# fperezgamonal/flownet2-tf

Measured on AMD Instinct MI355X. Metric: forward pairs/sec at 512x384 (FlowNet2), higher is better.
Workload: dtype f16x2 (split fp16 hi+lo operands, 3 fp16 MFMAs per product, fp32 accumulate); 1 GPU; FlowNet2 forward, batch=4 synthetic 512x384 pairs per GPU, seeded synthetic weights; pairs_per_gpu=4, parallelism=dp1 (no collective)

## Files before the change

flownet2-tf_amd/csrc/conv.hip:

```cpp
#include "conv_common.h"
#include <cstdlib>

namespace fn2 {

template <typename T, typename OutT, int TC, int WC, int WP>
__global__ void __launch_bounds__(256) conv_igemm_kernel(const ConvArgs p) {
  constexpr int CH = 16 / (int)sizeof(T);
  constexpr int BC = WC * TC * 16;
  constexpr int BP = WP * 64;
  constexpr int NT = 256;
  static_assert(WC * WP == 4, "4 waves per block");
  constexpr int NPR = BP / 64;
  constexpr int NWR = (BC * 4 + NT - 1) / NT;
  constexpr int WSWZ_BIT = (TC == 4) ? 5 : (TC == 2) ? 4 : 3;
  __shared__ uint4 lds[2][(BC + BP) * 4];

  const int tid = threadIdx.x, lane = tid & 63, wave = tid >> 6;
  const int wc = wave / WP, wp = wave % WP;
  const int cid = tid & 3;

  int pad_y = p.pad, pad_x = p.pad, oy_off = 0, ox_off = 0, osc = 1;
  const T* wgt = reinterpret_cast<const T*>(p.wgt);
  const int phase = blockIdx.z / p.splitk, split = blockIdx.z - phase * p.splitk;
  if (p.deconv) {
// ... 796 lines not shown
    plan->layout = 0; plan->cout_tile = 16; plan->kstep_elems = 64 / esz;
    plan->wgt_dtype = in_dtype == FN2_F16X2 ? FN2_F32 : in_dtype;
    return FN2_OK;
  }
  if (conv_fast_ok(in_dtype, cin_pad, cout)) {
    plan->layout = 1; plan->cout_tile = cout > 64 ? 128 : cout > 32 ? 64 : 32; plan->kstep_elems = 128 / esz;
    plan->wgt_dtype = in_dtype;
    return FN2_OK;
  }
  if (in_dtype == FN2_F16X2)
    return fail(FN2_ERR_UNSUPPORTED, "split-fp16 inputs need cin_pad %% 32 == 0 (LDS-DMA kernel); got %d", cin_pad);
  plan->layout = 0; plan->cout_tile = cout > 64 ? 128 : cout > 32 ? 64 : cout > 16 ? 32 : 16;
  plan->kstep_elems = 64 / esz; plan->wgt_dtype = in_dtype;
  return FN2_OK;
}

}

namespace fn2 {

static bool is_flow_head(const fn2_conv_desc* d) {
  return d->kind == 0 && d->out.c == 2 && d->kh == 3 && d->kw == 3 && d->stride == 1 && d->pad == 1 &&
         d->out.dtype == FN2_F32 && d->act == FN2_ACT_NONE;
}

static bool wants_bp64(const ConvArgs& a, int tile, int phases, int layout) {
  if (layout != 1 || (a.dbg & 32)) return false;
  if (tile < 128) return true;
  const char* e = getenv("FN2_BP64_MIN");
  const int min_blocks = e ? atoi(e) : 96;
  return cdiv(a.M, 64) * (long)(a.cout_pad / 128) * phases >= min_blocks;
}

static int build_args(const fn2_conv_desc* d, ConvArgs* out, int* tile_out, int* phases_out) {
  FN2_REQUIRE(d, "conv2d: null descriptor");
  int rc = check_view(&d->in, "conv2d input");
  if (rc) return rc;
  rc = check_view(&d->out, "conv2d output");
  if (rc) return rc;
  FN2_REQUIRE(d->wgt, "conv2d: null weights");
  FN2_REQUIRE((d->kind >= 0 && d->kind <= 3) || d->kind == 5,
              "conv2d: kind must be 0 (conv), 1 (deconv k4 s2 crop 1), 2 (stem row-run conv), 3 (transpose of a stride-2 conv) "
              "or 5 (deconv k4 s2 crop 1, column phases merged)");
  FN2_REQUIRE(d->in.n == d->out.n, "conv2d: batch mismatch");
  FN2_REQUIRE(d->up_src == nullptr || ((d->kind == 1 || d->kind == 5) && d->up_w != nullptr && d->up_c0 >= 0 &&
                                       d->up_c0 + 2 <= d->out.cs && !d->accumulate),
              "conv2d: up_src rides on a kind-1 / kind-5 transposed conv (up_w set, [up_c0, up_c0 + 2) inside the out buffer)");
  FN2_REQUIRE(d->cin_pad % 8 == 0 && d->cin_pad >= d->in.c, "conv2d: cin_pad must be a multiple of 8 >= Cin");
  FN2_REQUIRE(d->in.cs % 8 == 0 && d->in.c0 % 8 == 0, "conv2d: input channel stride/offset must be multiples of 8");
  if (d->kind != 2)
    FN2_REQUIRE(d->in.c0 + d->cin_pad <= d->in.cs, "conv2d: padded input channels exceed the buffer stride");
  const int esz = dtype_size(d->in.dtype);
  const int CH = 16 / esz;
  FN2_REQUIRE(d->kpad > 0 && d->kpad % (4 * CH) == 0, "conv2d: kpad must be a multiple of one k-step");
  fn2_conv_plan plan;
  rc = fn2_conv2d_plan(d->in.dtype, d->cin_pad, d->out.c, &plan);
  if (rc) return rc;
  const bool wfrag = d->wgt_layout == 2;
  if (wfrag)
    FN2_REQUIRE(plan.layout == 1 && plan.cout_tile >= 64 && d->in.dtype == FN2_F16X2 && d->kind != 2,
                "conv2d: wgt_layout 2 (fragment order) is for split-fp16 layers with more than 32 output channels");
  else
    FN2_REQUIRE(d->wgt_layout == plan.layout, "conv2d: wgt_layout %d does not match fn2_conv2d_plan (%d)", d->wgt_layout,
                plan.layout);
  const int tile = plan.cout_tile;
  FN2_REQUIRE(d->cout_pad % tile == 0 && d->cout_pad >= d->out.c, "conv2d: cout_pad must be a multiple of the cout tile");
  FN2_REQUIRE(d->act == FN2_ACT_NONE || d->act == FN2_ACT_LEAKY, "conv2d: bad activation");
  FN2_REQUIRE(d->out.dtype == d->in.dtype || d->out.dtype == FN2_F32 ||
                  (d->in.dtype == FN2_F32 && d->out.dtype == FN2_F16X2),
              "conv2d: output dtype must be the input dtype, fp32, or split-fp16 from an fp32 stem");
  if (d->in.dtype == FN2_F16X2) FN2_REQUIRE(d->in.cs % 8 == 0 && d->in.c0 % 8 == 0, "conv2d: split-fp16 views are group (8) aligned");
  if (d->out.dtype == FN2_F16X2) FN2_REQUIRE(d->out.cs % 8 == 0 && d->out.c0 % 8 == 0, "conv2d: split-fp16 views are group (8) aligned");

  ConvArgs& a = *out;
  a = ConvArgs{};
  a.KH_KW_hint = 0;
  a.wfrag = wfrag ? 1 : 0;
  a.merged = d->kind == 5 ? 1 : 0;
  a.in = d->in.data; a.wgt = d->wgt; a.bias = d->bias; a.out = d->out.data;
  a.N = d->in.n; a.H = d->in.h; a.W = d->in.w; a.in_cs = d->in.cs; a.in_c0 = d->in.c0;
// ... 109 lines not shown
  }
  a.kg = 1;
  if (d->wgt_layout == 1 && tile == 128 && !(a.dbg & 32)) {
    const char* e_kg = getenv("FN2_KG");
    if (!e_kg || atoi(e_kg) != 0) {
      const char* e3 = getenv("FN2_KG3_MAX");
      const char* e2 = getenv("FN2_KG2_MAX");
      const long blocks = (long)cdiv(a.M, 64) * (a.cout_pad / 128) * phases;
      if (blocks <= (e3 ? atoi(e3) : 0)) { a.bp64 = 1; a.kg = 3; }
      else if (blocks <= (e2 ? atoi(e2) : 95)) { a.bp64 = 1; a.kg = 2; }
    }
  }
  if (d->wgt_layout == 1 && tile == 128 && !(a.dbg & 32) && d->in.dtype == FN2_F16X2) {
    const char* e_lo = getenv("FN2_DEEP_MIN");
    const char* e_hi = getenv("FN2_DEEP_MAX");
    const long blocks = (long)cdiv(a.M, 64) * (a.cout_pad / 128) * phases;
    const int lo = e_lo ? atoi(e_lo) : 0, hi = e_hi ? atoi(e_hi) : -1;
    if (blocks >= lo && blocks <= hi) { a.bp64 = 3; a.kg = 1; }
  }
  if (d->wgt_layout == 1 && tile == 128 && a.bp64 == 1 && a.kg == 1) {
    const char* e_ring = getenv("FN2_RING_MAX");
    const int ring_max = e_ring ? atoi(e_ring) : 512;
    const long blocks = (long)cdiv(a.M, 64) * (a.cout_pad / 128) * phases;
    if ((a.dbg & 256) || (blocks >= 384 && blocks <= ring_max)) a.bp64 = 2;
    const char* e_rs = getenv("FN2_RING_SPLIT");
    if (e_rs && blocks >= atoi(e_rs) && blocks < 384) a.bp64 = 2;
  }
  *tile_out = tile;
  *phases_out = phases;
  return FN2_OK;
}

static int preferred_split(const ConvArgs& a, int tile, int phases) {
  if (a.merged) return 1;
  const int bp = tile == 128 ? (a.bp64 ? 64 : 128) : (a.bp64 ? 128 : 256);
  const long blocks = (long)cdiv(a.M, bp) * (a.cout_pad / tile) * phases;
  const char* e_min = getenv("FN2_SPLIT_MINBLOCKS");
  if (blocks >= (e_min ? atoi(e_min) : 384)) return 1;
  if (a.bp64 == 3) {
    const char* e_sl = getenv("FN2_DEEP_SLOTS");
    int s = (int)((e_sl ? atoi(e_sl) : 256) / blocks);
    const int maxs = a.ksteps / 16;
    if (s > maxs) s = maxs;
    if (s > 16) s = 16;
    if (s < 2) return 1;
    const int kper = cdiv(a.ksteps, s);
    return cdiv(a.ksteps, kper);
  }
  if (a.kg > 1) {
    const char* e_nos = getenv("FN2_KG_NOSPLIT");
    if (blocks >= (e_nos ? atoi(e_nos) : 96)) return 1;
    const char* e_sl = getenv("FN2_KG_SLOTS");
    int s = (int)((e_sl ? atoi(e_sl) : 256) / blocks);
    const int maxs = a.ksteps / (12 * a.kg);
    if (s > maxs) s = maxs;
    if (s > 16) s = 16;
    if (s < 2) return 1;
    const int kper = cdiv(a.ksteps, s);
    return cdiv(a.ksteps, kper);
  }
  const char* e = getenv("FN2_SPLIT_SLOTS");
  const char* e_rsl = getenv("FN2_RING_SPLIT_SLOTS");
  const int slots = (tile == 128 && a.bp64 == 2) ? (e_rsl ? atoi(e_rsl) : 512) : e ? atoi(e) : 640;
  int s = (int)(slots / blocks);
  const int maxs = a.ksteps / 8;
  if (s > maxs) s = maxs;
  if (s > 16) s = 16;
// ... 20 lines not shown
}

int fn2_conv2d_splits(const fn2_conv_desc* d) {
  ConvArgs a;
  int tile, phases;
  if (build_args(d, &a, &tile, &phases) != FN2_OK || is_flow_head(d)) return 1;
  int sk = preferred_split(a, tile, phases);
  while (sk > 1 && (d->workspace == nullptr || split_bytes(a, sk) > d->workspace_bytes)) --sk;
  if ((long)a.N * a.out_H * a.out_W * a.ws_cs >= (1L << 31)) sk = 1;
  if (sk > 1) {
    const int kper = cdiv(a.ksteps, sk);
    sk = cdiv(a.ksteps, kper);
    if (d->wgt_layout >= 1) sk = cdiv(a.ksteps / 2, cdiv(kper, 2));
  }
  return sk < 1 ? 1 : sk;
}

int fn2_conv2d_kernel_name(const fn2_conv_desc* d, char* name, int cap) {
  FN2_REQUIRE(name && cap > 0, "conv2d_kernel_name: no buffer");
  name[0] = 0;
  if (!d || d->wgt_layout < 1 || is_flow_head(d)) return FN2_OK;
  conv_name_sink() = ConvNameSink{name, cap};
  const int rc = fn2_conv2d(d, nullptr);
  conv_name_sink() = ConvNameSink{nullptr, 0};
  return rc;
}

int fn2_conv2d(const fn2_conv_desc* d, void* stream) {
  ConvArgs a;
  int tile, phases;
  int rc = build_args(d, &a, &tile, &phases);
  if (rc) return rc;
  hipStream_t s = (hipStream_t)stream;
  if (is_flow_head(d)) {
    int blocks = grid_for((long)a.M * 64, 256);
    if (d->in.dtype == FN2_F16X2 && a.M <= 4096 && !(a.dbg & 32768)) {
      a.dbg |= 16384;
      blocks = a.M;
    } else {
      a.dbg &= ~16384;
    }
    if (d->in.dtype == FN2_F32)
      hipLaunchKernelGGL(flow_head_kernel<float>, dim3(blocks), dim3(256), 0, s, a);
    else if (d->in.dtype == FN2_BF16)
      hipLaunchKernelGGL(flow_head_kernel<bf16_t>, dim3(blocks), dim3(256), 0, s, a);
    else if (d->in.dtype == FN2_F16)
      hipLaunchKernelGGL(flow_head_kernel<f16_t>, dim3(blocks), dim3(256), 0, s, a);
    else
      hipLaunchKernelGGL(flow_head_kernel<x2_t>, dim3(blocks), dim3(256), 0, s, a);
    FN2_CHECK_LAUNCH("flow_head");
    return FN2_OK;
  }
  int sk = preferred_split(a, tile, phases);
  while (sk > 1 && (d->workspace == nullptr || split_bytes(a, sk) > d->workspace_bytes)) --sk;
  if ((long)a.N * a.out_H * a.out_W * a.ws_cs >= (1L << 31)) sk = 1;
  if (sk > 1) {
    a.kper = cdiv(a.ksteps, sk);
    sk = cdiv(a.ksteps, a.kper);
  }
  if (sk > 1) {
    a.splitk = sk;
    a.ws = reinterpret_cast<float*>(d->workspace);
  }
  if (d->up_src != nullptr && d->kind == 5 && 2 * d->out.c == 32) {
    a.up_src = d->up_src; a.up_w = d->up_w; a.up_bias = d->up_bias; a.up_c0 = d->up_c0;
  }
// ... 248 lines not shown
```

flownet2-tf_amd/csrc/conv2.hip:

```cpp
#include "conv_common.h"

#include <type_traits>
#include <algorithm>
#include <utility>

#ifndef FN2_X2_ORDER
#define FN2_X2_ORDER 0
#endif
#ifndef FN2_CONV_ABLATE
#define FN2_CONV_ABLATE 0
#endif
#ifndef FN2_SETPRIO
#define FN2_SETPRIO 1
#endif

namespace fn2 {

typedef __attribute__((address_space(3))) void* lptr_t;

constexpr unsigned kOobOffset = 0x80000000u;

typedef int v4i_t __attribute__((ext_vector_type(4)));
typedef unsigned u32x4_t __attribute__((ext_vector_type(4)));

// ... 932 lines not shown
        for (int i = 0; i < 4; ++i) {
          const int row = i * 8 + rr;
          *reinterpret_cast<uint4*>(ob + (size_t)row * osc * p.out_cs) = *reinterpret_cast<const uint4*>(etl + row * ERS + ch * 4);
        }
      } else if (vec16 && cout_base + 15 < p.Cout) {
        store16<OutT>(po, v);
      } else {
#pragma unroll
        for (int q = 0; q < 16; ++q)
          if (cout_base + q < p.Cout) store_elem<OutT>(po + q, v[q]);
      }
      if (p.merged && p.up_src != nullptr && cout_base == 0 && ox < p.OW) {
        const int uy = toy * osc + oy_off, ux = ox * osc + ox_off + bsel;
        const int H2 = p.out_H >> 1, W2 = p.out_W >> 1;
        const int a = uy & 1, b = ux & 1, y = uy >> 1, x = ux >> 1;
        float r0 = p.up_bias ? p.up_bias[0] : 0.f, r1 = p.up_bias ? p.up_bias[1] : 0.f;
#pragma unroll
        for (int ty = 0; ty < 2; ++ty) {
          const int iy = y - 1 + a + ty, ky = 3 - a - 2 * ty;
          if (iy < 0 || iy >= H2) continue;
#pragma unroll
          for (int tx = 0; tx < 2; ++tx) {
            const int ix = x - 1 + b + tx, kx = 3 - b - 2 * tx;
            if (ix < 0 || ix >= W2) continue;
            const float2 sv = *reinterpret_cast<const float2*>(p.up_src + (((long)tn * H2 + iy) * W2 + ix) * 2);
            const float* ww = p.up_w + (ky * 4 + kx) * 4;
            r0 += sv.x * ww[0] + sv.y * ww[1];
            r1 += sv.x * ww[2] + sv.y * ww[3];
          }
        }
        OutT* pu = out + (((size_t)tn * p.out_H + uy) * p.out_W + ux) * p.out_cs + p.up_c0;
        store_elem<OutT>(pu, r0);
        store_elem<OutT>(pu + 1, r1);
      }
    }
  }
#endif
}

template <typename OutT, int NST>
__global__ void __launch_bounds__(256) conv_stem_kernel(const ConvArgs p, const int ntiles) {
#if defined(__HIP_DEVICE_COMPILE__)
  using T = x2_t;
  constexpr int ESZ = 4;
  constexpr int BC = 64, BP = 128, TCN = 2;
  __shared__ uint4 ldsA[NST][BC * 8];
  __shared__ uint4 ldsB[2][NST][BP * 8];
  const int tid = threadIdx.x, lane = tid & 63;
  const int wave = __builtin_amdgcn_readfirstlane(tid >> 6);
  const unsigned wrow_bytes = (unsigned)p.ksteps * 128u;
  const v4i_t rsrc_w = make_rsrc(p.wgt, (int)(p.cout_pad * wrow_bytes));
  const v4i_t rsrc_x = make_rsrc(p.in, p.in_bytes);
  const int lrow = lane >> 3, lphys = lane & 7;
  const int spt = p.cin_chunks >> 3;
#pragma unroll
  for (int st = 0; st < NST; ++st) {
    const int sc = st / p.KH, ky = st - sc * p.KH;
#pragma unroll
    for (int j = 0; j < 2; ++j) {
      const int row = wave * 16 + j * 8 + lrow;
      const unsigned woff = (unsigned)row * wrow_bytes + (unsigned)((lphys ^ ((row >> 1) & 7)) * 16);
      dma16(rsrc_w, &ldsA[st][(wave * 16 + j * 8) * 8], woff, (ky * spt + sc) * 128);
    }
  }
  auto issue_B = [&](int tile, int buf) {
#pragma unroll
// ... 526 lines not shown
        else if (a.wfrag == 2)
          hipLaunchKernelGGL((conv_igemm2_kernel<T, OutT, 4, 1, 1, 2, 3, 1, false, true, false>), grid, dim3(256), 0, s, a);
        else if (slab)
          hipLaunchKernelGGL((conv_igemm2_kernel<T, OutT, 4, 1, 1, 2, 2, 1, false, true, true>), grid, dim3(256), 0, s, a);
        else
          hipLaunchKernelGGL((conv_igemm2_kernel<T, OutT, 4, 1, 1, 2, 2, 1, false, true, false>), grid, dim3(256), 0, s, a);
      }
    } else {
      return fail(FN2_ERR_UNSUPPORTED, "conv fast path: fragment-order weights are split fp16 only");
    }
  } else if (tile == 128 && a.bp64 && a.kg == 3) FN2_LAUNCH2(cdiv(a.M, 64), a.cout_pad / 128, 768, 2, 2, 2, 1, 2, 3);
  else if (tile == 128 && a.bp64 && a.kg == 2) FN2_LAUNCH2(cdiv(a.M, 64), a.cout_pad / 128, 512, 2, 2, 2, 1, 2, 2);
  else if (tile == 128 && a.bp64 == 3) FN2_LAUNCH2(cdiv(a.M, 64), a.cout_pad / 128, 256, 2, 2, 2, 1, 6, 1);
  else if (tile == 128 && a.bp64 == 2) FN2_LAUNCH2(cdiv(a.M, 64), a.cout_pad / 128, 256, 2, 2, 2, 1, 3, 1);
  else if (tile == 128 && a.bp64) FN2_LAUNCH2(cdiv(a.M, 64), a.cout_pad / 128, 256, 2, 2, 2, 1, 2, 1);
  else if (tile == 128) FN2_LAUNCH2(cdiv(a.M, 128), a.cout_pad / 128, 256, 2, 2, 2, 2, 2, 1);
  else if (tile == 64 && a.bp64) FN2_LAUNCH2(cdiv(a.M, 128), a.cout_pad / 64, 256, 1, 4, 2, 1, 2, 1);
  else if (tile == 64) FN2_LAUNCH2(cdiv(a.M, 256), a.cout_pad / 64, 256, 1, 4, 2, 2, 2, 1);
  else if (a.bp64) FN2_LAUNCH2(cdiv(a.M, 128), a.cout_pad / 32, 256, 1, 4, 1, 1, 2, 1);
  else FN2_LAUNCH2(cdiv(a.M, 256), a.cout_pad / 32, 256, 1, 4, 1, 2, 2, 1);
#undef FN2_LAUNCH2
  FN2_CHECK_LAUNCH("conv_igemm2");
  return FN2_OK;
}

int launch_head5_strip(const ConvArgs& a, int blocks, hipStream_t s) {
  if (a.ksteps == 3) hipLaunchKernelGGL((head5_strip_kernel<1>), dim3(blocks), dim3(512), 0, s, a);
  else if (a.ksteps == 6) hipLaunchKernelGGL((head5_strip_kernel<2>), dim3(blocks), dim3(512), 0, s, a);
  else return fail(FN2_ERR_UNSUPPORTED, "flow_head5 strip form: %d channel lines (3 or 6)", a.ksteps);
  FN2_CHECK_LAUNCH("flow_head5_strip");
  return FN2_OK;
}

int launch_head5(const ConvArgs& a, int blocks, hipStream_t s) {
  hipLaunchKernelGGL((conv_igemm2_kernel<x2_t, float, 1, 4, 2, 2, 2, 1, false, false, false, true>), dim3(blocks, 1, 1), dim3(256), 0,
                     s, a);
  FN2_CHECK_LAUNCH("flow_head5");
  return FN2_OK;
}

bool conv_fast_ok(int in_dtype, int cin_pad, int cout) {
  const int esz = dtype_size(in_dtype);
  return cout > 2 && (cin_pad * esz) % 128 == 0;
}

int launch_conv_fast(const ConvArgs& a, int in_dtype, int out_dtype, int tile, int phases, hipStream_t s) {
  if (tile != 128 && tile != 64 && tile != 32) return fail(FN2_ERR_UNSUPPORTED, "conv fast path: cout tile %d", tile);
  if (in_dtype == FN2_F32) return launch2<float, float>(a, tile, phases, s);
  if (in_dtype == FN2_BF16) {
    if (out_dtype == FN2_BF16) return launch2<bf16_t, bf16_t>(a, tile, phases, s);
    return launch2<bf16_t, float>(a, tile, phases, s);
  }
  if (in_dtype == FN2_F16) {
    if (out_dtype == FN2_F16) return launch2<f16_t, f16_t>(a, tile, phases, s);
    return launch2<f16_t, float>(a, tile, phases, s);
  }
  if (out_dtype == FN2_F16X2) {
    if (launch_rowrun<x2_t>(a, tile, phases, s)) { FN2_CHECK_LAUNCH("conv_rowrun"); return FN2_OK; }
    if (launch_stem<x2_t>(a, tile, phases, s)) { FN2_CHECK_LAUNCH("conv_stem"); return FN2_OK; }
    if (launch_halo<x2_t>(a, tile, phases, s)) { FN2_CHECK_LAUNCH("conv_halo"); return FN2_OK; }
    if (a.merged) return fail(FN2_ERR_UNSUPPORTED, "conv2d kind 5: needs the halo kernel (input width a multiple of 128, no split-K)");
    return launch2<x2_t, x2_t>(a, tile, phases, s);
  }
  if (launch_halo<float>(a, tile, phases, s)) { FN2_CHECK_LAUNCH("conv_halo"); return FN2_OK; }
  if (a.merged) return fail(FN2_ERR_UNSUPPORTED, "conv2d kind 5: needs the halo kernel (input width a multiple of 128, no split-K)");
  return launch2<x2_t, float>(a, tile, phases, s);
// ... 4 lines not shown
```

flownet2-tf_amd/csrc/conv_common.h:

```cpp
#pragma once
#include "fn2_common.h"

namespace fn2 {

struct ConvArgs {
  const void* in;
  const void* wgt;
  const float* bias;
  void* out;
  int N, H, W, in_cs, in_c0;
  int cin_chunks;
  int KH, KW, stride, pad;
  int OH, OW;
  int M;
  int out_H, out_W, out_cs, out_c0, Cout;
  int ksteps;
  int cout_pad;
  int act;
  int deconv;
  int ph_pad0, ph_pad1;
  int kh_ph[2], kw_ph[2];
  int merged;
  int wmajor;
  int bp64;
  int KH_KW_hint;
  int kg;
  int h5_tx, h5_ty, h5_ring;
  int h5_tiles, h5_groups;
  const float* h5_wc;
  const float* h5_bc;
  int h5_rows;
  int fh_M, fh_z0;
  const float* fh_w;
  int fh_w1, fh_groups;
  const float* fh_bias;
  float* fh_out;
  int fh_out_cs, fh_out_c0;
  float fh_scale;
  const float* up_src; const float* up_w; const float* up_bias; int up_c0;
  int wfrag;
  int accum;
  int vec_ok;
  int splitk;
  int kper;
  float* ws;
  int ws_cs;
  float out_scale;
  int in_bytes;
  const void* mask_y;
  int mask_c0, mask_c1;
  int dbg;
};

__device__ __forceinline__ void fh_pixel(const x2_t* __restrict__ in, int H, int W, int in_cs, int in_c0, int groups,
                                         const float* __restrict__ wf0, const float* __restrict__ wf1,
// ... 56 lines not shown
#pragma unroll
        for (int q = 0; q < 16; ++q) v[q] += o[q];
      }
      if (mask) {
        float y[16];
        load16<OutT>(reinterpret_cast<const OutT*>(p.mask_y) + (po - out_base), y);
#pragma unroll
        for (int q = 0; q < 16; ++q)
          if (cout_base + q >= p.mask_c0 && cout_base + q < p.mask_c1) v[q] *= y[q] > 0.f ? 1.f : (y[q] < 0.f ? 0.1f : 0.55f);
      }
    } else {
#pragma unroll
      for (int q = 0; q < 16; ++q)
        if (cout_base + q < p.Cout) {
          if (p.accum) v[q] += load_elem<OutT>(po + q);
          v[q] = act_grad<OutT>(p, out_base, po + q, cout_base + q, v[q]);
        }
    }
  }
}

template <typename OutT>
__device__ __forceinline__ void store4(OutT* p, float a, float b, float c, float d) {
  const float v[4] = {a, b, c, d};
  store_vec<OutT, 4>(p, v);
}

struct ConvNameSink { char* buf; int cap; };
ConvNameSink& conv_name_sink();

int launch_conv_fast(const ConvArgs& a, int in_dtype, int out_dtype, int tile, int phases, hipStream_t s);
int launch_head5(const ConvArgs& a, int blocks, hipStream_t s);
int launch_head5_strip(const ConvArgs& a, int blocks, hipStream_t s);
bool conv_fast_ok(int in_dtype, int cin_pad, int cout);

}
```

flownet2-tf_amd/src/engine.py:

```python
import ctypes as C
import math
import os

import numpy as np
import torch

from . import _hip, netdefs, weights as W

_DT = {"f32": torch.float32, "bf16": torch.bfloat16, "f16": torch.float16, "f16x2": torch.float32}
_CODE = {"f32": _hip.FN2_F32, "bf16": _hip.FN2_BF16, "f16": _hip.FN2_F16, "f16x2": _hip.FN2_F16X2}
_TILE_ARGS = {128: "2, 2, 2, 2", 64: "1, 4, 2, 2", 32: "1, 4, 1, 2"}


def conv2_kernel_args(tile, m, cout_pad, phases, x2=True):
    dbg = int(os.environ.get("FN2_CONV_DBG", "0"))
    blocks64 = -(-m // 64) * (cout_pad // 128) * phases if tile == 128 else 0
    big = "FN2_M16_MIN" in os.environ and blocks64 >= max(int(os.environ["FN2_M16_MIN"]), 513)
    m16 = "true" if (x2 and not dbg & 512 and (dbg & 1024 or big)) else "false"
    full = dbg & 32
    if tile < 128:
        base = {64: "1, 4, 2, 2, 2, 1", 32: "1, 4, 1, 2, 2, 1"}[tile] if full else {64: "1, 4, 2, 1, 2, 1", 32: "1, 4, 1, 1, 2, 1"}[tile]
        return f"{base}, {m16}"
    blocks = -(-m // 64) * (cout_pad // 128) * phases
    if not full and int(os.environ.get("FN2_KG", "1")):
# ... 168 lines not shown
                eng._branch = self_.prev
        return _L()

    def _head_lane(self):
        hd = self._branch + 2
        return hd if (self._lanes_on and self._branch in (0, 1) and (self._lane_mask >> hd) & 1) else self._branch

    def _op(self, name, fn, *args, kernel=None):
        self.kernel_of.append(kernel if kernel is not None else fn.__name__.replace("fn2_", ""))
        self.ops.append((name, fn, args))
        self.branch_of.append(self._branch)

    def _conv(self, scope, spec, src, dst, up=None, up_after=None, defer_head=False):
        name, kind, k, stride, pad, cin, cout, act = spec
        sbuf, sc0, sc = src
        dbuf, dc0, dc = dst
        assert sc == cin and dc == cout, (scope, name, sc, cin, dc, cout)
        head_px = dbuf.shape[0] * dbuf.shape[1] * dbuf.shape[2]
        if (self.heads_as_gemm and kind == "conv" and cout == 2 and k == 3 and stride == 1 and pad == 1 and not act
                and dbuf.dtype == torch.float32 and head_px >= int(os.environ.get("FN2_HEAD_GEMM_MIN", "8192"))
                and self._head_gemm(scope, spec, src, dst, up)):
            return up is not None and bool(int(os.environ.get("FN2_FUSE_UPFLOW", "1")))
        wname = f"{scope}/{name}/weights"
        in_code = self._code(sbuf)
        esz = 2 if in_code in (_hip.FN2_BF16, _hip.FN2_F16) else 4
        cin_pad = _round_up(cin, 8)
        cin_line = _round_up(cin, 128 // esz)
        if sc0 + cin_line <= sbuf.shape[3] and _hip.conv_plan(in_code, cin_line, cout).layout == 1:
            cin_pad = cin_line
        plan = _hip.conv_plan(in_code, cin_pad, cout)
        tile, layout = plan.cout_tile, plan.layout
        merged = (kind != "conv" and self.compose_heads and cout == 16 and in_code == _hip.FN2_F16X2 and layout == 1
                  and tile == 32 and sbuf.shape[2] % 128 == 0 and bool(int(os.environ.get("FN2_DECONV_MERGED", "1"))))
        if kind == "conv":
            packed, cin_pad, cout_pad, kpad = W.pack_conv(self._w(wname), tile, plan.kstep_elems, cin_pad, layout)
        elif merged:
            packed, cin_pad, cout_pad, kpad = W.pack_deconv_merged(self._w(wname), tile, plan.kstep_elems, cin_pad, layout)
        else:
            packed, cin_pad, cout_pad, kpad = W.pack_deconv(self._w(wname), tile, plan.kstep_elems, cin_pad, layout)
        bias = self._bias(scope, name, kind, cout)
        out_scale = 1.0
        if plan.wgt_dtype == _hip.FN2_F16X2:
            wmax = float(abs(packed).max())
            if wmax > 0:
                k2 = int(math.floor(math.log2(1024.0 / wmax)))
                packed = packed * (2.0 ** k2)
                out_scale = 2.0 ** (-k2)
        wdev = W.packed_to_device(packed, plan.wgt_dtype, self.device)
        d = _hip.Fn2ConvDesc()
        d.inp = self._v(sbuf, sc, sc0)
        d.out = self._v(dbuf, dc, dc0)
        d.wgt = wdev.data_ptr()
        d.bias = bias.data_ptr() if bias is not None else None
        d.kind = 0 if kind == "conv" else (5 if merged else 1)
        d.kh = d.kw = k
        d.stride, d.pad = stride, pad
        d.act = _hip.ACT_LEAKY if act else _hip.ACT_NONE
        d.cin_pad, d.cout_pad, d.kpad = cin_pad, cout_pad, kpad
        d.wgt_layout = layout
        d.out_scale = out_scale
        frag = False
        if (self.fragment_weights and layout == 1 and tile >= int(os.environ.get("FN2_WREG_TILE_MIN", "128"))
                and plan.wgt_dtype == _hip.FN2_F16X2 and self._wants_fragments(d)):
            wdev = W.to_fragment_order(wdev)
            d.wgt, d.wgt_layout, frag = wdev.data_ptr(), 2, True
        self.keep += [d, wdev, bias]
        self.conv_descs.append(d)
        self.desc_branch.append(self._branch)
        up_rec = None
        if self._pending_head is not None and kind != "conv":
            hd = self._pending_head
            assert up_after is not None and hd.inp.data == d.inp.data and hd.inp.c0 == d.inp.c0, (scope, name)
            d.head = C.addressof(hd)
            self._pending_head = None
        if up_after is not None:
            assert kind != "conv" and (not merged or cout == 16)
            up_name, up_src, (ubuf, uc0, uc) = up_after
            assert ubuf is dbuf and uc == 2
            uw = W.to_device(self._w(f"{scope}/{up_name}/weights"), torch.float32, self.device)
            ub = self._bias(scope, up_name, "deconv", 2)
            d.up_src, d.up_w, d.up_bias, d.up_c0 = up_src.data_ptr(), uw.data_ptr(), (ub.data_ptr() if ub is not None else None), uc0
            uv = self._v(ubuf, uc, uc0)
            self.keep += [uw, ub, uv]
            up_rec = dict(scope=scope, name=up_name, kind="upflow", src=up_src, dst=up_after[2], w=uw, b=ub, view=uv)
        self.layers.append(dict(scope=scope, name=name, kind=d.kind, k=k, stride=stride, pad=pad, cin=cin, cout=cout,
                                act=bool(act), src=src, dst=dst, desc=d, w=wdev, b=bias, cin_pad=cin_pad,
                                cout_pad=cout_pad, kpad=kpad, layout=layout, tile=tile, kstep=plan.kstep_elems, frag=frag))
        if up_rec is not None:
            self.layers.append(up_rec)
        tn = _TNAME[self.dtype_name] if in_code == self.act_code else "float"
        if kind == "conv" and cout == 2 and k == 3 and stride == 1 and pad == 1:
            kern = f"flow_head_kernel<{tn}>"
# ... 735 lines not shown
```

flownet2-tf_amd/src/weights.py:

```python
import os

import numpy as np
import torch

from . import netdefs


def init_weights(model, seed=1234, flow_gain=0.25, bias_std=0.02, head_biases=None):
    if head_biases is None:
        head_biases = model != "FlowNetS_interp"
    rng = np.random.default_rng(seed)
    w = {}
    for scope, layers in netdefs.model_scopes(model):
        for (name, kind, k, stride, pad, cin, cout, act) in layers:
            if kind == "conv":
                fan_in = k * k * cin
                std = np.sqrt((2.0 if act else 1.0) / fan_in)
                if name.startswith("predict_flow"):
                    std *= flow_gain
                w[f"{scope}/{name}/weights"] = (rng.standard_normal((k, k, cin, cout)) * std).astype(np.float32)
                b = (rng.standard_normal((cout,)) * bias_std).astype(np.float32)
                if netdefs.has_bias(model, name, kind, not head_biases):
                    w[f"{scope}/{name}/biases"] = b
            else:
# ... 92 lines not shown
    cout_pad = _round_up(cout, cout_tile)
    kpad = _round_up(4 * cin_pad, kstep_elems)
    out = np.zeros((4, cout_pad, kpad), dtype)
    for a in range(2):
        for b in range(2):
            p = np.zeros((cout_pad, 4, cin_pad), dtype)
            for ty in range(2):
                for tx in range(2):
                    p[:cout, ty * 2 + tx, :cin] = w_hwoi[3 - a - 2 * ty, 3 - b - 2 * tx]
            ph = np.zeros((cout_pad, kpad), dtype)
            ph[:, :4 * cin_pad] = p.reshape(cout_pad, -1)
            out[a * 2 + b] = _permute_rows64(ph) if layout == 1 else ph
    return out, cin_pad, cout_pad, kpad


def pack_deconv_merged(w_hwoi, cout_tile, kstep_elems, cin_pad, layout=1, dtype=np.float32):
    kh, kw, cout, cin = w_hwoi.shape
    assert kh == 4 and kw == 4 and cout in (16, 32) and cin_pad >= cin and cin_pad % 8 == 0 and cout_tile == 32
    cout_pad = 2 * cout
    kpad = _round_up(6 * cin_pad, kstep_elems)
    out = np.zeros((2, cout_pad, kpad), dtype)
    for a in range(2):
        p = np.zeros((cout_pad, 6, cin_pad), dtype)
        for b in range(2):
            for ty in range(2):
                for tx in range(2):
                    p[b * cout:(b + 1) * cout, ty * 3 + b + tx, :cin] = w_hwoi[3 - a - 2 * ty, 3 - b - 2 * tx]
        ph = np.zeros((cout_pad, kpad), dtype)
        ph[:, :6 * cin_pad] = p.reshape(cout_pad, -1)
        out[a] = _permute_rows64(ph) if layout == 1 else ph
    return out, cin_pad, cout_pad, kpad


def pack_conv_transpose_s2(w_hwio, p, cout_tile, kstep_elems, cin_pad, layout, dtype=np.float32):
    k, _, ci, co = w_hwio.shape
    T = (k + 1) // 2
    cout_pad = _round_up(ci, cout_tile)
    kpad = _round_up(T * T * cin_pad, kstep_elems)
    assert cin_pad >= co

    def ceil_half(v):
        return -((-v) // 2)

    out = np.zeros((4, cout_pad, kpad), dtype)
    for a in range(2):
        lo_a = ceil_half(a + p - k + 1)
        for b in range(2):
            lo_b = ceil_half(b + p - k + 1)
            ph = np.zeros((cout_pad, T * T, cin_pad), dtype)
            for ty in range(T):
                ky = a + p - 2 * lo_a - 2 * ty
                if not 0 <= ky < k:
                    continue
                for tx in range(T):
                    kx = b + p - 2 * lo_b - 2 * tx
                    if 0 <= kx < k:
                        ph[:ci, ty * T + tx, :co] = w_hwio[ky, kx]
            full = np.zeros((cout_pad, kpad), dtype)
            full[:, :T * T * cin_pad] = ph.reshape(cout_pad, -1)
            out[a * 2 + b] = _permute_rows64(full) if layout == 1 else full
    return out, cin_pad, cout_pad, kpad


def to_device(arr, dtype, device):
    return torch.from_numpy(np.ascontiguousarray(arr)).to(device=device, dtype=dtype).contiguous()

# ... 55 lines not shown
```

Before: 1095 pairs/s.

## Add four-phase deconv kernel sharing one input tile across phases

Adds a new kind-6 transposed-conv kernel for the 4x4 stride-2 deconvs with 16 or 32 outputs. Each of the four waves computes one output phase from a shared LDS input halo tile, with all weights held in registers. The kernel is persistent, uses an XCD-aware tile order and a multi-slot DMA ring over channel chunks, and fuses the flow upsample into its epilogue. It replaces the merged or per-phase deconv paths by default, which cuts repeated input loads and launches at the cost of heavy register pressure and one block per CU.

```diff
diff --git a/flownet2-tf_amd/csrc/conv.hip b/flownet2-tf_amd/csrc/conv.hip
--- a/flownet2-tf_amd/csrc/conv.hip
+++ b/flownet2-tf_amd/csrc/conv.hip
@@ -852,6 +852,50 @@
   return cdiv(a.M, 64) * (long)(a.cout_pad / 128) * phases >= min_blocks;
 }
 
+static int build_args_deconv4p(const fn2_conv_desc* d, ConvArgs* out, int* tile_out, int* phases_out) {
+  FN2_REQUIRE(d->kh == 4 && d->kw == 4 && d->stride == 2, "deconv (kind 6): only k=4 s=2 crop 1");
+  FN2_REQUIRE((d->out.c == 16 || d->out.c == 32) && d->cout_pad == d->out.c,
+              "deconv (kind 6): 16 or 32 output channels, cout_pad = Cout");
+  FN2_REQUIRE(d->in.dtype == FN2_F16X2 && d->out.dtype == FN2_F16X2, "deconv (kind 6): split-fp16 input and output");
+  FN2_REQUIRE(d->wgt_layout == 3, "deconv (kind 6): wgt_layout must be 3 (weights.pack_deconv4p fragment order)");
+  FN2_REQUIRE(d->cin_pad % 32 == 0 && d->cin_pad >= d->in.c && d->in.c0 + d->cin_pad <= d->in.cs,
+              "deconv (kind 6): cin_pad must be whole 128-byte channel lines inside the input buffer");
+  FN2_REQUIRE(d->kpad == 16 * d->cin_pad, "deconv (kind 6): kpad must be 16 cin_pad (4 phases x 4 taps)");
+  FN2_REQUIRE(d->cin_pad == 64 || d->cin_pad == 128 || (d->cin_pad == 192 && d->out.c == 16),
+              "deconv (kind 6): cin_pad must be 64, 128 or 192 (16 output channels) / 64 or 128 (32)");
+  FN2_REQUIRE(d->in.cs % 8 == 0 && d->in.c0 % 8 == 0 && d->out.cs % 8 == 0 && d->out.c0 % 8 == 0,
+              "deconv (kind 6): split-fp16 views are group (8) aligned");
+  FN2_REQUIRE(d->out.h == 2 * d->in.h && d->out.w == 2 * d->in.w, "deconv: output must be 2H x 2W");
+  FN2_REQUIRE(d->act == FN2_ACT_NONE || d->act == FN2_ACT_LEAKY, "conv2d: bad activation");
+  FN2_REQUIRE(!d->accumulate && d->act_grad_y == nullptr && d->head == nullptr && !d->raw_partials,
+              "deconv (kind 6): no accumulate, act_grad_y, head or raw partials");
+  const long in_bytes = (long)d->in.n * d->in.h * d->in.w * d->in.cs * 4;
+  FN2_REQUIRE(in_bytes < (1L << 31), "conv2d: input buffer >= 2 GiB is not addressable by the LDS-DMA kernel");
+  FN2_REQUIRE((long)d->out.n * d->out.h * d->out.w * d->out.cs < (1L << 31), "conv2d: output buffer too large");
+  ConvArgs& a = *out;
+  a = ConvArgs{};
+  a.d4p = 1;
+  a.in = d->in.data; a.wgt = d->wgt; a.bias = d->bias; a.out = d->out.data;
+  a.N = d->in.n; a.H = d->in.h; a.W = d->in.w; a.in_cs = d->in.cs; a.in_c0 = d->in.c0;
+  a.cin_chunks = d->cin_pad / 4;
+  a.KH = 2; a.KW = 2; a.stride = 1; a.pad = 0;
+  a.OH = d->in.h; a.OW = d->in.w;
+  a.M = a.N * a.OH * a.OW;
+  a.deconv = 1; a.ph_pad0 = 1; a.ph_pad1 = 0;
+  a.out_H = d->out.h; a.out_W = d->out.w; a.out_cs = d->out.cs; a.out_c0 = d->out.c0; a.Cout = d->out.c;
+  a.ksteps = d->kpad / 16;
+  a.cout_pad = d->cout_pad;
+  a.act = d->act;
+  a.out_scale = d->out_scale == 0.f ? 1.f : d->out_scale;
+  a.vec_ok = 1;
+  a.splitk = 1; a.kper = a.ksteps; a.ws = nullptr; a.ws_cs = (a.Cout + 3) / 4 * 4;
+  a.in_bytes = (int)in_bytes;
+  if (d->up_src != nullptr) { a.up_src = d->up_src; a.up_w = d->up_w; a.up_bias = d->up_bias; a.up_c0 = d->up_c0; }
+  *tile_out = d->out.c;
+  *phases_out = 4;
+  return FN2_OK;
+}
+
 static int build_args(const fn2_conv_desc* d, ConvArgs* out, int* tile_out, int* phases_out) {
   FN2_REQUIRE(d, "conv2d: null descriptor");
   int rc = check_view(&d->in, "conv2d input");
@@ -859,13 +903,14 @@
   rc = check_view(&d->out, "conv2d output");
   if (rc) return rc;
   FN2_REQUIRE(d->wgt, "conv2d: null weights");
-  FN2_REQUIRE((d->kind >= 0 && d->kind <= 3) || d->kind == 5,
-              "conv2d: kind must be 0 (conv), 1 (deconv k4 s2 crop 1), 2 (stem row-run conv), 3 (transpose of a stride-2 conv) "
-              "or 5 (deconv k4 s2 crop 1, column phases merged)");
+  FN2_REQUIRE((d->kind >= 0 && d->kind <= 3) || d->kind == 5 || d->kind == 6,
+              "conv2d: kind must be 0 (conv), 1 (deconv k4 s2 crop 1), 2 (stem row-run conv), 3 (transpose of a stride-2 conv), "
+              "5 (deconv k4 s2 crop 1, column phases merged) or 6 (deconv k4 s2 crop 1, four phases in one block)");
   FN2_REQUIRE(d->in.n == d->out.n, "conv2d: batch mismatch");
-  FN2_REQUIRE(d->up_src == nullptr || ((d->kind == 1 || d->kind == 5) && d->up_w != nullptr && d->up_c0 >= 0 &&
+  FN2_REQUIRE(d->up_src == nullptr || ((d->kind == 1 || d->kind == 5 || d->kind == 6) && d->up_w != nullptr && d->up_c0 >= 0 &&
                                        d->up_c0 + 2 <= d->out.cs && !d->accumulate),
-              "conv2d: up_src rides on a kind-1 / kind-5 transposed conv (up_w set, [up_c0, up_c0 + 2) inside the out buffer)");
+              "conv2d: up_src rides on a kind-1 / 5 / 6 transposed conv (up_w set, [up_c0, up_c0 + 2) inside the out buffer)");
+  if (d->kind == 6) return build_args_deconv4p(d, out, tile_out, phases_out);
   FN2_REQUIRE(d->cin_pad % 8 == 0 && d->cin_pad >= d->in.c, "conv2d: cin_pad must be a multiple of 8 >= Cin");
   FN2_REQUIRE(d->in.cs % 8 == 0 && d->in.c0 % 8 == 0, "conv2d: input channel stride/offset must be multiples of 8");
   if (d->kind != 2)
@@ -1041,7 +1086,7 @@
 }
 
 static int preferred_split(const ConvArgs& a, int tile, int phases) {
-  if (a.merged) return 1;
+  if (a.merged || a.d4p) return 1;
   const int bp = tile == 128 ? (a.bp64 ? 64 : 128) : (a.bp64 ? 128 : 256);
   const long blocks = (long)cdiv(a.M, bp) * (a.cout_pad / tile) * phases;
   const char* e_min = getenv("FN2_SPLIT_MINBLOCKS");
@@ -1128,6 +1173,7 @@
   int rc = build_args(d, &a, &tile, &phases);
   if (rc) return rc;
   hipStream_t s = (hipStream_t)stream;
+  if (a.d4p) return launch_deconv4p(a, s);
   if (is_flow_head(d)) {
     int blocks = grid_for((long)a.M * 64, 256);
     if (d->in.dtype == FN2_F16X2 && a.M <= 4096 && !(a.dbg & 32768)) {
diff --git a/flownet2-tf_amd/csrc/conv2.hip b/flownet2-tf_amd/csrc/conv2.hip
--- a/flownet2-tf_amd/csrc/conv2.hip
+++ b/flownet2-tf_amd/csrc/conv2.hip
@@ -988,6 +988,194 @@
         OutT* pu = out + (((size_t)tn * p.out_H + uy) * p.out_W + ux) * p.out_cs + p.up_c0;
         store_elem<OutT>(pu, r0);
         store_elem<OutT>(pu + 1, r1);
+      }
+    }
+  }
+#endif
+}
+
+constexpr int D4_BP = 64;
+constexpr int d4_ty(int U) { return U == 1 ? 2 : 1; }
+constexpr int d4_depth(int NCH) { return NCH % 3 == 0 ? 3 : 4; }
+
+template <int U, int NCH>
+__global__ void __launch_bounds__(256, 1) deconv4p_kernel(const ConvArgs p) {
+#if defined(__HIP_DEVICE_COMPILE__)
+  constexpr int TY = d4_ty(U), BP = D4_BP, RW = BP + 2;
+  constexpr int NE = (TY + 2) * RW, NPC = (NE + 7) / 8, NPW = (NPC + 3) / 4;
+  constexpr int CT = BP / 16;
+  constexpr int NF = 8 * U;
+  constexpr int D = NCH < d4_depth(NCH) ? NCH : d4_depth(NCH);
+  constexpr int SLOT = 4 * NPW * 64;
+  static_assert(NCH % D == 0, "ring slots divide the chunks: the slot of a chunk is static");
+  __shared__ uint4 lds[D * SLOT];
+
+  const int tid = threadIdx.x, lane = tid & 63;
+  const int wave = __builtin_amdgcn_readfirstlane(tid >> 6);
+  const int pa = wave >> 1, pb = wave & 1;
+  const int ntx = (p.W + BP - 1) / BP, nty = (p.H + TY - 1) / TY, ntiles = p.N * nty * ntx;
+  const int G = gridDim.x;
+  int b0 = blockIdx.x;
+  {
+    const int xcd = b0 & 7, chunk = G >> 3, rem = G & 7;
+    b0 = xcd * chunk + min(xcd, rem) + (b0 >> 3);
+  }
+  const int nmine = b0 < ntiles ? (ntiles - 1 - b0) / G + 1 : 0;
+  if (nmine == 0) return;
+
+  const v4i_t rsrc_x = make_rsrc(p.in, p.in_bytes);
+  const int j8 = lane >> 3, cg = (j8 & 4) | ((j8 & 1) << 1) | ((j8 >> 1) & 1);
+  auto tile_xy = [&](int t, int& n, int& y0, int& x0) __attribute__((always_inline)) {
+    x0 = (t % ntx) * BP;
+    const int q = t / ntx;
+    y0 = (q % nty) * TY;
+    n = q / nty;
+  };
+  auto tile_offsets = [&](int t, unsigned (&bo)[NPW]) __attribute__((always_inline)) {
+    int n, y0, x0;
+    tile_xy(t, n, y0, x0);
+#pragma unroll
+    for (int j = 0; j < NPW; ++j) {
+      const int q = wave + 4 * j, e = 8 * q + (lane & 7);
+      const int r = e / RW, c = e - r * RW, iy = y0 - 1 + r, ix = x0 - 1 + c;
+      const bool ok = q < NPC && e < NE && iy >= 0 && iy < p.H && ix >= 0 && ix < p.W;
+      bo[j] = ok ? (unsigned)((((n * p.H + iy) * p.W + ix) * p.in_cs + p.in_c0) * 4 + cg * 16) : kOobOffset;
+    }
+  };
+  auto issue = [&](const unsigned (&bo)[NPW], int s, uint4* slot) __attribute__((always_inline)) {
+#pragma unroll
+    for (int j = 0; j < NPW; ++j) dma16(rsrc_x, &slot[(wave + 4 * j) * 64], bo[j] + (unsigned)s * 128u, 0);
+  };
+
+  uint4 w[NCH][NF];
+  {
+    const uint4* src = reinterpret_cast<const uint4*>(p.wgt) + (size_t)wave * NF * 64 + lane;
+#pragma unroll
+    for (int s = 0; s < NCH; ++s)
+#pragma unroll
+      for (int f = 0; f < NF; ++f) w[s][f] = src[(size_t)s * (4 * NF * 64) + f * 64];
+  }
+  const int l15 = lane & 15, kq = lane >> 4;
+  float bias[U][4];
+#pragma unroll
+  for (int u = 0; u < U; ++u)
+#pragma unroll
+    for (int i = 0; i < 4; ++i) bias[u][i] = p.bias != nullptr ? p.bias[16 * u + 4 * kq + i] : 0.f;
+
+  const int hs = (kq >> 1) * 4 + (kq & 1);
+  f32x4 acc[TY * CT][U];
+  auto compute = [&](const uint4* B, const uint4 (&wf)[NF]) __attribute__((always_inline)) {
+#if FN2_SETPRIO
+    __builtin_amdgcn_s_setprio(1);
+#endif
+#pragma unroll
+    for (int t = 0; t < TY * CT; ++t) {
+      const int r = t / CT, c = t - r * CT;
+#pragma unroll
+      for (int tap = 0; tap < 4; ++tap) {
+        const int ty = tap >> 1, tx = tap & 1;
+        const int e = (r + ty + pa) * RW + 16 * c + tx + pb + l15;
+        const uint4* src = B + ((e >> 3) * 64 + hs * 8 + (e & 7));
+        const uint4 bh = src[0], bl = src[16];
+#pragma unroll
+        for (int u = 0; u < U; ++u) {
+          const uint4 ah = wf[(tap * U + u) * 2], al = wf[(tap * U + u) * 2 + 1];
+          acc[t][u] = mfma_16x16x32<f16_t>(al, bh, acc[t][u]);
+          acc[t][u] = mfma_16x16x32<f16_t>(ah, bl, acc[t][u]);
+          acc[t][u] = mfma_16x16x32<f16_t>(ah, bh, acc[t][u]);
+        }
+      }
+    }
+#if FN2_SETPRIO
+    __builtin_amdgcn_s_setprio(0);
+#endif
+  };
+
+  x2_t* out = reinterpret_cast<x2_t*>(p.out);
+  auto epilogue = [&](int tile) __attribute__((always_inline)) {
+    int n, y0, x0;
+    tile_xy(tile, n, y0, x0);
+#pragma unroll
+    for (int u = 0; u < U; ++u) {
+      const int cb = 16 * u + 4 * kq;
+#pragma unroll
+      for (int t = 0; t < TY * CT; ++t) {
+        const int r = t / CT, c = t - r * CT;
+        const int iy = y0 + r, ix = x0 + 16 * c + l15;
+        if (iy >= p.H || ix >= p.W) continue;
+        x2_t* po = out + (((size_t)n * p.out_H + (2 * iy + pa)) * p.out_W + (2 * ix + pb)) * p.out_cs + p.out_c0 + cb;
+        float v[4];
+#pragma unroll
+        for (int i = 0; i < 4; ++i) v[i] = acc[t][u][i] * p.out_scale + bias[u][i];
+        if (p.act == FN2_ACT_LEAKY) {
+#pragma unroll
+          for (int i = 0; i < 4; ++i) v[i] = leaky(v[i]);
+        }
+        store_vec<x2_t, 4>(po, v);
+      }
+    }
+  };
+
+  unsigned bo_cur[NPW], bo_next[NPW];
+  tile_offsets(b0, bo_cur);
+#pragma unroll
+  for (int s = 0; s < D - 1; ++s) issue(bo_cur, s, &lds[s * SLOT]);
+  for (int it = 0; it < nmine; ++it) {
+    const int tile = b0 + it * G;
+    const bool has_next = it + 1 < nmine;
+    if (has_next) tile_offsets(tile + G, bo_next);
+#pragma unroll
+    for (int t = 0; t < TY * CT; ++t)
+#pragma unroll
+      for (int u = 0; u < U; ++u) acc[t][u] = f32x4{0.f, 0.f, 0.f, 0.f};
+    [&]<int... S>(std::integer_sequence<int, S...>) __attribute__((always_inline)) {
+      ([&]() __attribute__((always_inline)) {
+        constexpr int s = S;
+        constexpr int ahead = (D - 2) < (NCH - 1 - s) ? (D - 2) : (NCH - 1 - s);
+        if (has_next) asm volatile("s_waitcnt vmcnt(%0)\n\ts_barrier" :: "n"(NPW * (D - 2)) : "memory");
+        else asm volatile("s_waitcnt vmcnt(%0)\n\ts_barrier" :: "n"(NPW * ahead) : "memory");
+        constexpr int s2 = s + D - 1;
+        if constexpr (s2 < NCH) issue(bo_cur, s2, &lds[(s2 % D) * SLOT]);
+        else if (has_next) issue(bo_next, s2 - NCH, &lds[(s2 % D) * SLOT]);
+        compute(&lds[(s % D) * SLOT], w[s]);
+      }(), ...);
+    }(std::make_integer_sequence<int, NCH>{});
+    epilogue(tile);
+    if (has_next) {
+#pragma unroll
+      for (int j = 0; j < NPW; ++j) bo_cur[j] = bo_next[j];
+    }
+  }
+
+  if (p.up_src != nullptr) {
+    const int H2 = p.out_H >> 1, W2 = p.out_W >> 1;
+    for (int it = 0; it < nmine; ++it) {
+      int n, y0, x0;
+      tile_xy(b0 + it * G, n, y0, x0);
+#pragma unroll
+      for (int k = 0; k < TY * BP / 64; ++k) {
+        const int px = lane + 64 * k, iy = y0 + px / BP, ix = x0 + px % BP;
+        if (iy >= p.H || ix >= p.W) continue;
+        const int uy = 2 * iy + pa, ux = 2 * ix + pb;
+        const int a = uy & 1, b = ux & 1, y = uy >> 1, x = ux >> 1;
+        float r0 = p.up_bias ? p.up_bias[0] : 0.f, r1 = p.up_bias ? p.up_bias[1] : 0.f;
+#pragma unroll
+        for (int ty = 0; ty < 2; ++ty) {
+          const int yy = y - 1 + a + ty, ky = 3 - a - 2 * ty;
+          if (yy < 0 || yy >= H2) continue;
+#pragma unroll
+          for (int tx = 0; tx < 2; ++tx) {
+            const int xx = x - 1 + b + tx, kx = 3 - b - 2 * tx;
+            if (xx < 0 || xx >= W2) continue;
+            const float2 sv = *reinterpret_cast<const float2*>(p.up_src + (((long)n * H2 + yy) * W2 + xx) * 2);
+            const float* ww = p.up_w + (ky * 4 + kx) * 4;
+            r0 += sv.x * ww[0] + sv.y * ww[1];
+            r1 += sv.x * ww[2] + sv.y * ww[3];
+          }
+        }
+        x2_t* pu = out + (((size_t)n * p.out_H + uy) * p.out_W + ux) * p.out_cs + p.up_c0;
+        store_elem<x2_t>(pu, r0);
+        store_elem<x2_t>(pu + 1, r1);
       }
     }
   }
@@ -1580,6 +1768,33 @@
   return FN2_OK;
 }
 
+int launch_deconv4p(const ConvArgs& a, hipStream_t s) {
+  const int U = a.Cout / 16, nch = a.cin_chunks >> 3;
+  if (conv_name_sink().buf) {
+    snprintf(conv_name_sink().buf, conv_name_sink().cap, "deconv4p_kernel<%d, %d>", U, nch);
+    return FN2_OK;
+  }
+  static int cus = 0;
+  if (cus == 0) {
+    int dev = 0, n = 0;
+    cus = (hipGetDevice(&dev) == hipSuccess &&
+           hipDeviceGetAttribute(&n, hipDeviceAttributeMultiprocessorCount, dev) == hipSuccess && n > 0) ? n : 256;
+  }
+  const int ty = d4_ty(U);
+  const long tiles = (long)a.N * ((a.H + ty - 1) / ty) * ((a.W + D4_BP - 1) / D4_BP);
+  const dim3 grid((unsigned)std::min<long>(tiles, cus));
+#define FN2_D4P(UU, NN) hipLaunchKernelGGL((deconv4p_kernel<UU, NN>), grid, dim3(256), 0, s, a)
+  if (U == 1 && nch == 2) FN2_D4P(1, 2);
+  else if (U == 1 && nch == 4) FN2_D4P(1, 4);
+  else if (U == 1 && nch == 6) FN2_D4P(1, 6);
+  else if (U == 2 && nch == 2) FN2_D4P(2, 2);
+  else if (U == 2 && nch == 4) FN2_D4P(2, 4);
+  else return fail(FN2_ERR_UNSUPPORTED, "conv2d kind 6: %d output channels x %d channel lines", a.Cout, nch);
+#undef FN2_D4P
+  FN2_CHECK_LAUNCH("deconv4p");
+  return FN2_OK;
+}
+
 int launch_head5(const ConvArgs& a, int blocks, hipStream_t s) {
   hipLaunchKernelGGL((conv_igemm2_kernel<x2_t, float, 1, 4, 2, 2, 2, 1, false, false, false, true>), dim3(blocks, 1, 1), dim3(256), 0,
                      s, a);
diff --git a/flownet2-tf_amd/csrc/conv_common.h b/flownet2-tf_amd/csrc/conv_common.h
--- a/flownet2-tf_amd/csrc/conv_common.h
+++ b/flownet2-tf_amd/csrc/conv_common.h
@@ -21,6 +21,7 @@
   int ph_pad0, ph_pad1;
   int kh_ph[2], kw_ph[2];
   int merged;
+  int d4p;
   int wmajor;
   int bp64;
   int KH_KW_hint;
@@ -143,6 +144,7 @@
 int launch_conv_fast(const ConvArgs& a, int in_dtype, int out_dtype, int tile, int phases, hipStream_t s);
 int launch_head5(const ConvArgs& a, int blocks, hipStream_t s);
 int launch_head5_strip(const ConvArgs& a, int blocks, hipStream_t s);
+int launch_deconv4p(const ConvArgs& a, hipStream_t s);
 bool conv_fast_ok(int in_dtype, int cin_pad, int cout);
 
 }
diff --git a/flownet2-tf_amd/src/engine.py b/flownet2-tf_amd/src/engine.py
--- a/flownet2-tf_amd/src/engine.py
+++ b/flownet2-tf_amd/src/engine.py
@@ -224,8 +224,14 @@
         tile, layout = plan.cout_tile, plan.layout
         merged = (kind != "conv" and self.compose_heads and cout == 16 and in_code == _hip.FN2_F16X2 and layout == 1
                   and tile == 32 and sbuf.shape[2] % 128 == 0 and bool(int(os.environ.get("FN2_DECONV_MERGED", "1"))))
+        four = (kind != "conv" and self.compose_heads and cout in (16, 32) and in_code == _hip.FN2_F16X2
+                and self._code(dbuf) == _hip.FN2_F16X2 and cin_pad in ((64, 128, 192) if cout == 16 else (64, 128))
+                and bool(int(os.environ.get("FN2_DECONV4P", "1"))))
+        merged = merged and not four
         if kind == "conv":
             packed, cin_pad, cout_pad, kpad = W.pack_conv(self._w(wname), tile, plan.kstep_elems, cin_pad, layout)
+        elif four:
+            packed, cin_pad, cout_pad, kpad = W.pack_deconv4p(self._w(wname), cin_pad)
         elif merged:
             packed, cin_pad, cout_pad, kpad = W.pack_deconv_merged(self._w(wname), tile, plan.kstep_elems, cin_pad, layout)
         else:
@@ -238,18 +244,18 @@
                 k2 = int(math.floor(math.log2(1024.0 / wmax)))
                 packed = packed * (2.0 ** k2)
                 out_scale = 2.0 ** (-k2)
-        wdev = W.packed_to_device(packed, plan.wgt_dtype, self.device)
+        wdev = W.to_deconv4p_fragments(packed, self.device) if four else W.packed_to_device(packed, plan.wgt_dtype, self.device)
         d = _hip.Fn2ConvDesc()
         d.inp = self._v(sbuf, sc, sc0)
         d.out = self._v(dbuf, dc, dc0)
         d.wgt = wdev.data_ptr()
         d.bias = bias.data_ptr() if bias is not None else None
-        d.kind = 0 if kind == "conv" else (5 if merged else 1)
+        d.kind = 0 if kind == "conv" else (6 if four else 5 if merged else 1)
         d.kh = d.kw = k
         d.stride, d.pad = stride, pad
         d.act = _hip.ACT_LEAKY if act else _hip.ACT_NONE
         d.cin_pad, d.cout_pad, d.kpad = cin_pad, cout_pad, kpad
-        d.wgt_layout = layout
+        d.wgt_layout = 3 if four else layout
         d.out_scale = out_scale
         frag = False
         if (self.fragment_weights and layout == 1 and tile >= int(os.environ.get("FN2_WREG_TILE_MIN", "128"))
diff --git a/flownet2-tf_amd/src/weights.py b/flownet2-tf_amd/src/weights.py
--- a/flownet2-tf_amd/src/weights.py
+++ b/flownet2-tf_amd/src/weights.py
@@ -148,6 +148,28 @@
     return out, cin_pad, cout_pad, kpad
 
 
+def pack_deconv4p(w_hwoi, cin_pad, dtype=np.float32):
+    kh, kw, cout, cin = w_hwoi.shape
+    assert kh == 4 and kw == 4 and cout in (16, 32) and cin_pad >= cin and cin_pad % 32 == 0
+    out = np.zeros((4, 4, cout, cin_pad), dtype)
+    for a in range(2):
+        for b in range(2):
+            for ty in range(2):
+                for tx in range(2):
+                    out[a * 2 + b, ty * 2 + tx, :, :cin] = w_hwoi[3 - a - 2 * ty, 3 - b - 2 * tx]
+    out = out.reshape(4, 4, cout // 16, 16, cin_pad // 32, 32).transpose(4, 0, 1, 2, 3, 5)
+    return np.ascontiguousarray(out), cin_pad, cout, 16 * cin_pad
+
+
+def to_deconv4p_fragments(packed, device):
+    s = split_f16x2(packed)
+    lead = s.shape[:-2]
+    s = s.reshape(lead + (16, 4, 2, 8))
+    n = len(lead)
+    s = s.transpose(tuple(range(n)) + (n + 2, n + 1, n, n + 3))
+    return torch.from_numpy(np.ascontiguousarray(s)).to(device).contiguous()
+
+
 def pack_conv_transpose_s2(w_hwio, p, cout_tile, kstep_elems, cin_pad, layout, dtype=np.float32):
     k, _, ci, co = w_hwio.shape
     T = (k + 1) // 2
```

Result: no change. 1105 pairs/s, median of 6 (+1.0%).
